# adrelino/mv-lm-icp

Hardware: NVIDIA H100
Metric: ICP iterations/sec (corr+LM) (higher is better)
Workload: dtype f64

## Files before the change

### mv_lm_icp_b200/csrc/lm_step.cuh

```cuda
#pragma once
#include <cuda_runtime.h>
#include "../../include/mvicp.h"
#include "se3_math.cuh"
#include "types.cuh"

namespace mv {

constexpr int STEP_THREADS = 512;
constexpr int EOUT = 160;

struct LmState {
  mvicp_lm_options opt;
  int32_t param, cost_kind, robust, M, E, F, n, G;
  int32_t phase, done, termination, iteration, n_success, n_invalid, n_evals, n_solves, reuse_diagonal, nonrigid;
  double radius, decrease_factor, x_cost, cand_cost, x_norm, initial_cost, model_cost_change, step_norm, gmax;
};

struct NormalLayout {
  const int32_t* col;
  const int32_t* hb_ptr; const int32_t* hb_row; const int32_t* hb_col; const int32_t* hc_edge; const int32_t* hc_sub; int32_t n_hblocks;
  const int32_t* gb_ptr; const int32_t* gc_edge; const int32_t* gc_side;
  const int32_t* rlast; const int32_t* rfirst;
  const int32_t* rowbase;
  double *Lg, *rhs;
  int32_t l_in_smem;
  double* poses16;
  volatile int32_t* host_flag;
  int32_t seq;
};

struct LmWork {
  LmState* S;
  const EdgeDev* edges;
  const double* eout;
  volatile int* peer_flags;
  int32_t world, xseq;
  double* x;
  double* cand;
  Rt* Rt_eval;
  double* K_eval;
  FrameGen* G_eval;
  NormalLayout lay;
  double *H, *g, *Hc, *gc, *scale, *diag, *step;
  long long* prof;
};

struct LmProblem {
  LmState* S;
  const int32_t* frame;
  const int32_t* edge;
  NormalLayout lay;
  double *H, *g, *Hc, *gc, *scale, *diag, *step;
};

__device__ __forceinline__ double block_sum(double v, double* red) {
  __syncthreads();
  const int lane = threadIdx.x & 31, wid = threadIdx.x >> 5;
#pragma unroll
  for (int o = 16; o > 0; o >>= 1) v += __shfl_down_sync(0xffffffffu, v, o);
  if (lane == 0) red[wid] = v;
  __syncthreads();
  if (threadIdx.x == 0) { double s = 0; for (int w = 0; w < STEP_THREADS / 32; ++w) s += red[w]; red[32] = s; }
  __syncthreads();
  return red[32];
}
__device__ __forceinline__ double block_max(double v, double* red) {
  __syncthreads();
  const int lane = threadIdx.x & 31, wid = threadIdx.x >> 5;
#pragma unroll
  for (int o = 16; o > 0; o >>= 1) v = fmax(v, __shfl_down_sync(0xffffffffu, v, o));
  if (lane == 0) red[wid] = v;
  __syncthreads();
  if (threadIdx.x == 0) { double s = 0; for (int w = 0; w < STEP_THREADS / 32; ++w) s = fmax(s, red[w]); red[32] = s; }
  __syncthreads();
  return red[32];
}

__device__ __forceinline__ void gather_blocks(const NormalLayout& l, const double* eout, int n, double* H) {
  for (int idx = threadIdx.x; idx < l.n_hblocks * 36; idx += blockDim.x) {
    const int b = idx / 36, r = idx - 36 * b, i = r / 6, j = r - 6 * i;
    double s = 0;
    for (int c = l.hb_ptr[b]; c < l.hb_ptr[b + 1]; ++c) {
      const int e = l.hc_edge[c], sub = l.hc_sub[c];
      s += eout[(size_t)EOUT * e + (6 * (sub >> 1) + i) * 12 + 6 * (sub & 1) + j];
    }
    H[(size_t)(l.hb_row[b] + i) * n + l.hb_col[b] + j] = s;
  }
}
__device__ __forceinline__ void gather_gradient(const NormalLayout& l, const double* eout, int M, double* g) {
  for (int idx = threadIdx.x; idx < M * 6; idx += blockDim.x) {
    const int f = idx / 6, i = idx - 6 * f;
    if (l.col[f] < 0) continue;
    double s = 0;
    for (int c = l.gb_ptr[f]; c < l.gb_ptr[f + 1]; ++c) s += eout[(size_t)EOUT * l.gc_edge[c] + 144 + 6 * l.gc_side[c] + i];
    g[l.col[f] + i] = s;
  }
}
__device__ __forceinline__ double edge_cost_sum(const double* eout, int E, double* red, const int32_t* edge = nullptr) {
  double s = 0.0;
  for (int e = threadIdx.x; e < E; e += blockDim.x) s += eout[(size_t)EOUT * (edge ? edge[e] : e) + 156];
  return block_sum(s, red);
}
template <typename State> __device__ __forceinline__ void copy_state(State* dst, const State* src) {
  for (int i = threadIdx.x; i < (int)(sizeof(State) / sizeof(int32_t)); i += blockDim.x)
    reinterpret_cast<int32_t*>(dst)[i] = reinterpret_cast<const int32_t*>(src)[i];
  __syncthreads();
}
__device__ __forceinline__ void publish_step(const NormalLayout& l, bool done) {
  __threadfence();
  l.host_flag[l.seq & 7] = (l.seq << 1) | (done ? 1 : 0);
  __threadfence_system();
}

__global__ void lm_init_kernel(LmWork w) {
  LmState* S = w.S;
  const int f = blockIdx.x * blockDim.x + threadIdx.x;
  if (f >= S->M) return;
  double x[7] = {0, 0, 0, 0, 0, 0, 0};
  param_of_pose(S->param, w.lay.poses16 + 16 * f, x);
  if (S->param != PARAM_AA) {
    const double n2 = x[0] * x[0] + x[1] * x[1] + x[2] * x[2] + x[3] * x[3];
    if (!(fabs(n2 - 1.0) <= 1e-9)) atomicExch(&S->nonrigid, 1);
  }
  Rt a; Rt_of_param(S->param, x, &a);
  double K[36]; tangent_map(S->param, x, &a, K);
  for (int i = 0; i < 7; ++i) { w.x[7 * f + i] = x[i]; w.cand[7 * f + i] = x[i]; }
  w.Rt_eval[f] = a;
  for (int i = 0; i < 36; ++i) w.K_eval[36 * f + i] = K[i];
  if (w.G_eval && S->param != PARAM_AA) frame_general(S->param, x, &w.G_eval[f]);
}

__device__ __forceinline__ void chol_factor_diag(double* L, const int32_t* rb, int j0, double* dinv, volatile int* s_ok, int lane) {
  double D[6][6], inv[6];
#pragma unroll
  for (int i = 0; i < 6; ++i)
#pragma unroll
    for (int k = 0; k <= i; ++k) D[i][k] = L[rb[j0 + i] + j0 + k];
  bool okb = true;
#pragma unroll
  for (int k = 0; k < 6; ++k) {
    double d = D[k][k];
#pragma unroll
    for (int m = 0; m < k; ++m) d -= D[k][m] * D[k][m];
    if (!(d > 0.0) || !isfinite(d)) okb = false;
    inv[k] = rsqrt(d); D[k][k] = d * inv[k];
#pragma unroll
    for (int i = k + 1; i < 6; ++i) {
      double v = D[i][k];
#pragma unroll
      for (int m = 0; m < k; ++m) v -= D[i][m] * D[k][m];
      D[i][k] = v * inv[k];
    }
  }
  __syncwarp();
  if (lane == 0) {
    if (!okb) *s_ok = 0;
#pragma unroll
    for (int i = 0; i < 6; ++i) {
#pragma unroll
      for (int k = 0; k <= i; ++k) L[rb[j0 + i] + j0 + k] = D[i][k];
      dinv[j0 + i] = inv[i];
    }
  }
}

__device__ bool chol_solve(double* L, const int32_t* __restrict__ rowbase, int n, double* scratch, double* dinv, double* y,
                           const int32_t* __restrict__ rlast, const int32_t* __restrict__ rfirst, long long* prof = nullptr) {
  const int T = blockDim.x, tid = threadIdx.x, lane = tid & 31, wid = tid >> 5, nw = T >> 5;
  int32_t* s_rfirst = reinterpret_cast<int32_t*>(scratch);
  int32_t* s_rlast = s_rfirst + n;
  int32_t* rb = s_rlast + n;
  volatile int* s_ok = reinterpret_cast<volatile int*>(rb + n + 1);
  for (int i = tid; i < n; i += T) { s_rfirst[i] = rfirst[i]; s_rlast[i] = rlast[i]; }
  for (int i = tid; i <= n; i += T) rb[i] = rowbase[i];
  if (tid == 0) *s_ok = 1;
  __syncthreads();
  const int NB = n / 6;
  if (wid == 0) chol_factor_diag(L, rb, 0, dinv, s_ok, lane);
  __syncthreads();
  long long t_panel = 0, t_ahead = 0, t_bar = 0;
  for (int J = 0; J < NB; ++J) {
    if (!*s_ok) return false;
    const long long c0 = prof ? clock64() : 0;
    const int j0 = 6 * J;
    const int rl = s_rlast[j0 + 5];
    const int nrows = rl - (j0 + 5) + 1;
    for (int q = tid; q < nrows; q += T) {
      const int r = (q == nrows - 1) ? n : j0 + 6 + q;
      if (r < n && s_rfirst[r] > j0 + 5) continue;
      double* row = L + rb[r] + j0;
      double v[6];
#pragma unroll
      for (int k = 0; k < 6; ++k) {
        double a = row[k];
#pragma unroll
        for (int m = 0; m < k; ++m) a -= v[m] * L[rb[j0 + k] + j0 + m];
        v[k] = a * dinv[j0 + k];
      }
#pragma unroll
      for (int k = 0; k < 6; ++k) row[k] = v[k];
    }
    const long long c1 = prof ? clock64() : 0;
    __syncthreads();
    const long long c2 = prof ? clock64() : 0;
    const bool next = J + 1 < NB;
    if (wid == 0 && next) {
      const int b0 = j0 + 6;
      if (lane < 21 && s_rfirst[b0] <= j0 + 5) {
        int i = 0, rem = lane; while (rem > i) { rem -= i + 1; ++i; }
        const int k = rem;
        double* row = L + rb[b0 + i]; const double* lc = L + rb[b0 + k] + j0;
        double a = row[b0 + k];
#pragma unroll
        for (int m = 0; m < 6; ++m) a -= row[j0 + m] * lc[m];
        row[b0 + k] = a;
      }
      __syncwarp();
      chol_factor_diag(L, rb, b0, dinv, s_ok, lane);
    } else {
      const int w0 = next ? 1 : 0, wn = next ? nw - 1 : nw;
      const int qfirst = next ? 6 : 0;
      for (int q = qfirst + (wid - w0); q < nrows; q += wn) {
        const int r = (q == nrows - 1) ? n : j0 + 6 + q;
        if (r < n && s_rfirst[r] > j0 + 5) continue;
        double* row = L + rb[r];
        double lr[6];
#pragma unroll
        for (int k = 0; k < 6; ++k) lr[k] = row[j0 + k];
        const int cend = min(r, rl);
        for (int c = j0 + 6 + lane; c <= cend; c += 32) {
          if (s_rfirst[c] > j0 + 5) continue;
          const double* lc = L + rb[c] + j0;
          double a = row[c];
#pragma unroll
          for (int k = 0; k < 6; ++k) a -= lr[k] * lc[k];
          row[c] = a;
        }
      }
    }
    const long long c3 = prof ? clock64() : 0;
    __syncthreads();
    if (prof) { const long long c4 = clock64(); t_panel += c1 - c0; t_ahead += c3 - c2; t_bar += (c2 - c1) + (c4 - c3); }
  }
  if (prof && tid == 0) { prof[8] = t_panel; prof[9] = t_ahead; prof[10] = t_bar; }
  if (!*s_ok) return false;
  for (int i = tid; i < n; i += T) y[i] = L[rb[n] + i];
  __syncthreads();
  if (wid == 0) {
    for (int J = NB - 1; J >= 0; --J) {
      const int j0 = 6 * J;
      double x[6];
#pragma unroll
      for (int k = 5; k >= 0; --k) {
        double a = y[j0 + k];
#pragma unroll
        for (int m = k + 1; m < 6; ++m) a -= L[rb[j0 + m] + j0 + k] * x[m];
        x[k] = a * dinv[j0 + k];
      }
      __syncwarp();
#pragma unroll
      for (int k = 0; k < 6; ++k) if (lane == k) y[j0 + k] = x[k];
      for (int i = s_rfirst[j0] + lane; i < j0; i += 32) {
        double a = y[i];
#pragma unroll
        for (int k = 0; k < 6; ++k) a -= L[rb[j0 + k] + i] * x[k];
        y[i] = a;
      }
      __syncwarp();
    }
  }
  __syncthreads();
  return true;
}

template <bool COMP>
__device__ __forceinline__ void lm_step_body(const LmWork& w, const LmProblem& p) {
  extern __shared__ double smem[];
  __shared__ double red[40];
  __shared__ int s_flag;
  if (p.S->done) { if (!COMP && threadIdx.x == 0) publish_step(w.lay, true); return; }
  const int tid = threadIdx.x, T = blockDim.x;
  __shared__ LmState s_state;
  copy_state(&s_state, p.S);
  LmState* S = &s_state;
  const int n = S->n, M = S->M, E = S->E, param = S->param;
  const NormalLayout& lay = p.lay;
  auto gf = [&](int f) { return COMP ? p.frame[f] : f; };
  long long* prof = w.prof ? w.prof + 16 * (w.lay.seq & 3) : nullptr;
#define MV_STAMP(i) do { if (prof && tid == 0) prof[i] = clock64(); } while (0)
  MV_STAMP(0);
  if (w.peer_flags) {
    if (tid < w.world) {
      const long long t0 = clock64();
      while (w.peer_flags[tid] - w.xseq < 0) {
        if (clock64() - t0 > 4000000000LL) { S->nonrigid = 2; break; }
      }
    }
    __syncthreads();
  }
  double* colj = smem; double* dg = smem + 2 * (S->n + 1);
  double* L = lay.l_in_smem ? smem + 3 * (S->n + 1) : lay.Lg;

  gather_blocks(lay, w.eout, n, p.Hc);
  gather_gradient(lay, w.eout, M, p.gc);
  __syncthreads();
  const double eval_cost = edge_cost_sum(w.eout, E, red, COMP ? p.edge : nullptr);

  MV_STAMP(1);
  bool take = false;
  if (tid == 0) {
    s_flag = 0;
    S->n_evals += 1;
    if (!isfinite(eval_cost)) {
      if (S->phase == 0) { S->done = 1; S->termination = MVICP_TERM_EVAL_FAILURE; }
      else {
        S->n_invalid += 1;
        if (S->n_invalid >= S->opt.max_num_consecutive_invalid_steps) { S->done = 1; S->termination = MVICP_TERM_INVALID_STEPS; }
        S->radius = S->radius / S->decrease_factor; S->decrease_factor *= 2.0; S->reuse_diagonal = 1;
      }
    } else if (S->phase == 0) {
      S->x_cost = eval_cost; S->initial_cost = eval_cost; s_flag = 1;
    } else {
      S->cand_cost = eval_cost;
      if (S->step_norm <= S->opt.parameter_tolerance * (S->x_norm + S->opt.parameter_tolerance)) {
        S->done = 1; S->termination = MVICP_TERM_PARAMETER_TOLERANCE;
      } else if (fabs(S->x_cost - eval_cost) <= S->opt.function_tolerance * S->x_cost) {
        S->done = 1; S->termination = MVICP_TERM_FUNCTION_TOLERANCE;
      } else {
        const double rho = (S->x_cost - eval_cost) / S->model_cost_change;
        if (rho > S->opt.min_relative_decrease) {
          s_flag = 1; S->n_success += 1; S->x_cost = eval_cost;
          const double q = 2.0 * rho - 1.0;
          S->radius = fmin(S->opt.max_trust_region_radius, S->radius / fmax(1.0 / 3.0, 1.0 - q * q * q));
          S->decrease_factor = 2.0; S->reuse_diagonal = 0;
        } else {
          S->radius = S->radius / S->decrease_factor; S->decrease_factor *= 2.0; S->reuse_diagonal = 1;
          if (S->radius < S->opt.min_trust_region_radius) { S->done = 1; S->termination = MVICP_TERM_MIN_RADIUS; }
        }
      }
    }
  }
  __syncthreads();
  take = s_flag != 0;
  if (take) {
    for (int idx = tid; idx < lay.n_hblocks * 36; idx += T) {
      const int b = idx / 36, r = idx - 36 * b, i = r / 6, j = r - 6 * i;
      const size_t at = (size_t)(lay.hb_row[b] + i) * n + lay.hb_col[b] + j;
      p.H[at] = p.Hc[at];
    }
    for (int idx = tid; idx < n; idx += T) p.g[idx] = p.gc[idx];
    for (int idx = tid; idx < M * 7; idx += T) { const int at = COMP ? 7 * gf(idx / 7) + idx % 7 : idx; w.x[at] = w.cand[at]; }
    __syncthreads();
    if (S->phase == 0)
      for (int j = tid; j < n; j += T) p.scale[j] = S->opt.jacobi_scaling ? 1.0 / (1.0 + sqrt(p.H[(size_t)j * n + j])) : 1.0;
    double xs = 0.0, gm = 0.0;
    for (int f = tid; f < M; f += T) {
      if (lay.col[f] < 0) continue;
      const int G = S->G;
      double xf[7], ng[6], xp[7];
      for (int i = 0; i < G; ++i) { xf[i] = w.x[7 * gf(f) + i]; xs += xf[i] * xf[i]; }
      for (int i = 0; i < 6; ++i) ng[i] = -p.g[lay.col[f] + i];
      param_plus(param, xf, ng, xp);
      for (int i = 0; i < G; ++i) gm = fmax(gm, fabs(xf[i] - xp[i]));
    }
    xs = block_sum(xs, red);
    gm = block_max(gm, red);
    if (tid == 0) {
      S->x_norm = sqrt(xs); S->gmax = gm;
      if (gm <= S->opt.gradient_tolerance) { S->done = 1; S->termination = MVICP_TERM_GRADIENT_TOLERANCE; }
      if (S->phase == 0) { S->phase = 1; S->iteration = 0; S->reuse_diagonal = 0; }
    }
    __syncthreads();
  }

  MV_STAMP(2);
  while (!S->done) {
    __syncthreads();
    if (S->iteration >= S->opt.max_num_iterations) {
      __syncthreads();
      if (tid == 0) { S->done = 1; S->termination = MVICP_TERM_MAX_ITERATIONS; }
      __syncthreads();
      break;
    }
    const int reuse = S->reuse_diagonal;
    const double radius = S->radius;
    __syncthreads();
    if (!reuse)
      for (int j = tid; j < n; j += T) {
        const double d = p.scale[j] * p.scale[j] * p.H[(size_t)j * n + j];
        p.diag[j] = fmin(fmax(d, S->opt.min_lm_diagonal), S->opt.max_lm_diagonal);
      }
    __syncthreads();
    for (int i = tid >> 5; i < n; i += T >> 5) {
      const double si = p.scale[i];
      const int rbi = lay.rowbase[i];
      for (int j = lay.rfirst[i] + (tid & 31); j <= i; j += 32) {
        double v = si * p.H[(size_t)i * n + j] * p.scale[j];
        if (i == j) { const double ldg = sqrt(p.diag[i] / radius); v += ldg * ldg; }
        L[rbi + j] = v;
      }
    }
    { const int rbn = lay.rowbase[n]; for (int j = tid; j < n; j += T) L[rbn + j] = p.scale[j] * p.g[j]; }
    __syncthreads();
    MV_STAMP(3);
    bool ok = chol_solve(L, lay.rowbase, n, colj, dg, lay.rhs, lay.rlast, lay.rfirst, prof);
    MV_STAMP(4);
    double bad = 0.0;
    if (ok) for (int j = tid; j < n; j += T) if (!isfinite(lay.rhs[j])) bad = 1.0;
    bad = block_sum(bad, red);
    ok = ok && (bad == 0.0);
    double mcc = 0.0;
    if (ok) {
      for (int j = tid; j < n; j += T) p.step[j] = -lay.rhs[j];
      __syncthreads();
      double acc = 0.0;
      for (int i = tid; i < n; i += T) {
        const double y = lay.rhs[i];
        acc += 0.5 * (y * p.scale[i] * p.g[i] + (p.diag[i] / radius) * y * y);
      }
      mcc = block_sum(acc, red);
    }
    const bool valid = ok && (mcc > 0.0);
    __syncthreads();
    if (tid == 0) {
      S->iteration += 1; S->n_solves += 1; S->reuse_diagonal = 1; S->model_cost_change = mcc;
      if (!valid) {
        S->n_invalid += 1;
        if (S->n_invalid >= S->opt.max_num_consecutive_invalid_steps) { S->done = 1; S->termination = MVICP_TERM_INVALID_STEPS; }
        S->radius = S->radius / S->decrease_factor; S->decrease_factor *= 2.0;
      } else S->n_invalid = 0;
    }
    __syncthreads();
    if (!valid) continue;
    double sn = 0.0;
    for (int f = tid; f < M; f += T) {
      const int G = S->G, g_f = gf(f);
      double xf[7], d[6], xp[7] = {0, 0, 0, 0, 0, 0, 0};
      for (int i = 0; i < 7; ++i) xf[i] = w.x[7 * g_f + i];
      if (lay.col[f] >= 0) {
        for (int i = 0; i < 6; ++i) d[i] = p.step[lay.col[f] + i] * p.scale[lay.col[f] + i];
        param_plus(param, xf, d, xp);
        for (int i = 0; i < G; ++i) sn += (xf[i] - xp[i]) * (xf[i] - xp[i]);
      } else for (int i = 0; i < 7; ++i) xp[i] = xf[i];
      for (int i = 0; i < 7; ++i) w.cand[7 * g_f + i] = xp[i];
      Rt a; Rt_of_param(param, xp, &a);
      w.Rt_eval[g_f] = a;
      double K[36]; tangent_map(param, xp, &a, K);
      for (int i = 0; i < 36; ++i) w.K_eval[36 * g_f + i] = K[i];
      if (w.G_eval && param != PARAM_AA) frame_general(param, xp, &w.G_eval[g_f]);
    }
    sn = block_sum(sn, red);
    MV_STAMP(5);
    if (tid == 0) S->step_norm = sqrt(sn);
    __syncthreads();
    break;
  }
  __syncthreads();
  if (S->done) {
    for (int f = tid; f < M; f += T) {
      double xf[7]; for (int i = 0; i < 7; ++i) xf[i] = w.x[7 * gf(f) + i];
      pose_of_param(param, xf, w.lay.poses16 + 16 * gf(f));
    }
  }
  __syncthreads();
  copy_state(p.S, &s_state);
  MV_STAMP(6);
  if (!COMP && tid == 0) publish_step(w.lay, S->done);
  MV_STAMP(7);
#undef MV_STAMP
}

__global__ void __launch_bounds__(STEP_THREADS) lm_step_kernel(LmWork w) {
  const LmProblem p{w.S, nullptr, nullptr, w.lay, w.H, w.g, w.Hc, w.gc, w.scale, w.diag, w.step};
  lm_step_body<false>(w, p);
}

__global__ void __launch_bounds__(STEP_THREADS) lm_step_components_kernel(LmWork w, const LmProblem* __restrict__ probs, unsigned int* ticket) {
  __shared__ LmProblem s_prob;
  copy_state(&s_prob, probs + blockIdx.x);
  lm_step_body<true>(w, s_prob);
  __shared__ int s_last;
  __syncthreads();
  if (threadIdx.x == 0) { __threadfence(); s_last = atomicAdd(ticket, 1u) == gridDim.x - 1; }
  __syncthreads();
  if (!s_last) return;
  __threadfence();
  int open = 0;
  for (int k = threadIdx.x; k < (int)gridDim.x; k += blockDim.x) open |= *(volatile const int*)&probs[k].S->done == 0;
  open = __syncthreads_count(open);
  if (threadIdx.x == 0) { *ticket = 0u; publish_step(w.lay, open == 0); }
}

}
```

### mv_lm_icp_b200/csrc/mvicp.cu

```cuda
#include <cuda_runtime.h>
#include <nccl.h>
#ifdef __linux__
#include <sched.h>
#endif
#include <algorithm>
#include <atomic>
#include <cmath>
#include <cstdarg>
#include <cstdio>
#include <cstdlib>
#include <cstring>
#include <limits>
#include <numeric>
#include <string>
#include <thread>
#include <vector>

#include "../../include/mvicp.h"
#include "closed.cuh"
#include "compact.cuh"
#include "device_io.cuh"
#include "far.cuh"
#include "g2o.cuh"
#include "knn.cuh"
// ... 3 lines not shown
#include "se3_math.cuh"
#include "select.cuh"
#include "types.cuh"

using namespace mv;

static thread_local std::string g_err;
static int fail(int code, const char* fmt, ...) {
  char buf[512];
  va_list ap; va_start(ap, fmt); vsnprintf(buf, sizeof buf, fmt, ap); va_end(ap);
  g_err = buf;
  return code;
}
#define CU(call)                                                                                              \
  do {                                                                                                        \
    cudaError_t e_ = (call);                                                                                  \
    if (e_ != cudaSuccess) return fail(MVICP_ERR_CUDA, "%s:%d %s: %s", __FILE__, __LINE__, #call, cudaGetErrorString(e_)); \
  } while (0)
#define NC(call)                                                                                              \
  do {                                                                                                        \
    ncclResult_t r_ = (call);                                                                                 \
    if (r_ != ncclSuccess) return fail(MVICP_ERR_NCCL, "%s:%d %s: %s", __FILE__, __LINE__, #call, ncclGetErrorString(r_)); \
  } while (0)
#define RET(call) do { int r__ = (call); if (r__ != MVICP_OK) return r__; } while (0)

struct DevBuf {
  void* p = nullptr; size_t cap = 0;
  DevBuf() = default;
  DevBuf(const DevBuf&) = delete;
  DevBuf& operator=(const DevBuf&) = delete;
  ~DevBuf() { release(); }
  int reserve(size_t bytes) {
    if (bytes <= cap) return MVICP_OK;
    if (p) cudaFree(p);
    p = nullptr; cap = 0;
    CU(cudaMalloc(&p, bytes ? bytes : 16));
    cap = bytes ? bytes : 16;
    return MVICP_OK;
  }
  void release() { if (p) cudaFree(p); p = nullptr; cap = 0; }
  template <typename T> T* as() const { return reinterpret_cast<T*>(p); }
};

struct mvicp_ctx {
  int device = 0, flags = 0;
  cudaStream_t stream = nullptr; bool own_stream = false;
  int rank = 0, world = 1; ncclComm_t comm = nullptr;
  void* xbuf = nullptr; void* peer_x[MAX_PEERS] = {}; bool p2p_ok = false; int32_t xseq = 0;
  static constexpr int X_ECAP = 4096;
  int M = 0; bool f32 = true; bool nor_f32 = true; bool have_normals = true;
  std::vector<void*> nor_dbl;
  float normals_ms = 0.f;
  std::vector<int64_t> n_pts;
  std::vector<FrameDev> h_frames;
  std::vector<void*> frame_allocs;
  DevBuf d_obb;
  int seeded_rounds = 0;
  DevBuf d_single;
  DevBuf d_prof;
  DevBuf d_tile_count, d_tile_off, d_edge_off, d_recs;
  bool obb_ready = false;
  int last_lm_iters = 1 << 20;
  DevBuf d_frames, d_poses;
  std::vector<uint8_t> fixed;
  std::vector<double> h_poses;
  int E = 0;
  std::vector<EdgeDev> h_edges;
  std::vector<int32_t> edge_owner;
  DevBuf d_edges, d_xf, d_corr, d_d2, d_count, d_sel, d_hist, d_weight, d_median, d_selcand, d_selcand_n;
  DevBuf d_sel_cnt;
  DevBuf d_sel_win;
  DevBuf d_certs, d_cert_cnt;
  DevBuf d_todo, d_todo_n;
  bool cert_valid = false;
  int64_t cert_rounds = 0;
  bool sel_valid = false;
  int64_t sel_guess_rounds = 0;
  DevBuf d_knn_tiles, d_eval_tiles, d_edge_tile_begin, d_partial;
  int n_knn_tiles = 0, n_eval_tiles = 0, eval_tile_len = EVAL_TILE;
  int64_t total_slots = 0;
  bool have_corr = false;
  bool nonrigid = false;
  std::vector<float> h_weight; std::vector<unsigned long long> h_count;
  DevBuf d_state, d_x, d_cand, d_Rt, d_K, d_col, d_H, d_g, d_Hc, d_gc, d_scale, d_diag, d_L, d_rhs, d_step,
      d_eout, d_hb_ptr, d_hb_row, d_hb_col, d_hc_edge, d_hc_sub, d_gb_ptr, d_gc_edge, d_gc_side, d_posegather, d_rlast, d_rfirst, d_rowbase, d_gen;
  int64_t l_size = 0;
  int n_free = 0;
  NormalLayout lay{};
  std::vector<int32_t> h_col;
  void* h_state = nullptr;
  volatile int32_t* h_flag = nullptr; volatile int32_t* d_flag = nullptr;
  std::vector<uint8_t> lm_key; uint32_t graph_gen = 0;
  DevBuf d_cmp_i32, d_cmp_f64, d_cmp_prob, d_cmp_state, d_cmp_ticket;
  std::vector<uint8_t> cmp_key;
  std::vector<int32_t> cmp_of_frame;
  std::vector<int32_t> cmp_prob;
  std::vector<int32_t> cmp_M, cmp_E, cmp_n;
  int n_cmp = 0, n_prob = 0; size_t cmp_dyn = 0, cmp_edge_map = 0;
  DevBuf d_g2o_state, d_g2o_x, d_g2o_ev, d_g2o_nop, d_g2o_chi, d_g2o_trace, d_g2o_tiles, d_g2o_tile_begin, d_g2o_cnt;
  int64_t g2o_trials = 0;
  mvicp_stats stats{};
  cudaEvent_t ev[8]{};
  std::vector<cudaEvent_t> eval_ev;
  int eval_ev_used = 0;
  bool ev_knn = false, ev_lm = false;
  float lm_eval_acc = 0.f;
  DevBuf d_cpq, d_cpr;
  DevBuf d_set_win, d_set_bad;
  DevBuf d_knn_nor;
};

static inline int owner_of(const mvicp_ctx* c, int frame) { return (int)(((int64_t)frame * c->world) / std::max(1, c->M)); }
static void assign_edge_owners(mvicp_ctx* c) {
  const int E = c->E;
  c->edge_owner.assign(E, -1);
  int64_t total = 0;
  for (int e = 0; e < E; ++e) if (!c->fixed[c->h_edges[e].src]) total += c->n_pts[c->h_edges[e].src];
  int64_t before = 0;
  for (int e = 0; e < E; ++e) {
    const int s = c->h_edges[e].src;
    if (c->fixed[s]) continue;
    const int64_t n = c->n_pts[s];
    c->edge_owner[e] = total > 0 ? (int)std::min<int64_t>(c->world - 1, ((2 * before + n) * c->world) / (2 * total)) : 0;
    before += n;
  }
}

#include "tree_build.h"
#include "tree_gpu.cuh"

extern "C" { static int refresh_after_fixed_change(mvicp_ctx* c); }

static bool poses_nonrigid(const double* poses16, int M) {
  for (int f = 0; f < M; ++f) {
    Rt a; pose16_to_Rt(poses16 + 16 * f, &a);
    double q[4]; quat_of_matrix(a.R, q);
    const double n2 = q[0] * q[0] + q[1] * q[1] + q[2] * q[2] + q[3] * q[3];
    if (!(std::fabs(n2 - 1.0) <= 1e-9)) return true;
  }
  return false;
}

static unsigned host_workers() {
  unsigned n = std::max(1u, std::thread::hardware_concurrency());
#ifdef __linux__
  cpu_set_t set; CPU_ZERO(&set);
  if (sched_getaffinity(0, sizeof set, &set) == 0) { const int k = CPU_COUNT(&set); if (k > 0) n = std::min<unsigned>(n, (unsigned)k); }
  if (FILE* f = std::fopen("/sys/fs/cgroup/cpu.max", "r")) {
    char q[32]; long long period = 0;
    if (std::fscanf(f, "%31s %lld", q, &period) == 2 && std::strcmp(q, "max") != 0 && period > 0) {
      const long long quota = std::atoll(q);
      if (quota > 0) n = std::min<unsigned>(n, (unsigned)std::max<long long>(1, quota / period));
    }
    std::fclose(f);
  }
#endif
  return std::max(1u, n);
}

static int finish_set_frames(mvicp_ctx* c, int M) {
  if (c->f32 && c->nor_f32)
    for (int f = 0; f < M; ++f) {
      FrameDev& fr = c->h_frames[f];
      if (!fr.nor_o) continue;
      void* d_pn = nullptr;
      CU(cudaMalloc(&d_pn, sizeof(float4) * 2 * (size_t)fr.n)); c->frame_allocs.push_back(d_pn);
      pack_pn_kernel<<<(fr.n + 255) / 256, 256, 0, c->stream>>>((const float4*)fr.pts_o, (const float4*)fr.nor_o, fr.n, (float4*)d_pn);
// ... 956 lines not shown
        v = c->h_flag[want & 7];
        if ((v >> 1) != want) { CU(cudaGetLastError()); return fail(MVICP_ERR_CUDA, "%s step %d never reported", what, want); }
        break;
      }
    }
    ++seen;
    if ((v & 1) != 0 || seen > max_evals) break;
  }
  return MVICP_OK;
}

static int read_back_solve(mvicp_ctx* c, void* state, const void* d_state, size_t bytes) {
  CU(cudaEventRecord(c->ev[4], c->stream));
  CU(cudaMemcpyAsync(state, d_state, bytes, cudaMemcpyDeviceToHost, c->stream));
  CU(cudaMemcpyAsync(c->h_poses.data(), c->d_poses.p, sizeof(double) * 16 * c->M, cudaMemcpyDeviceToHost, c->stream));
  CU(cudaStreamSynchronize(c->stream));
  CU(cudaGetLastError());
  c->ev_lm = true;
  return MVICP_OK;
}

static int refresh_if_fixed_changed(mvicp_ctx* c) {
  bool stale = false;
  for (int e = 0; e < c->E; ++e) if ((c->edge_owner[e] < 0) != (c->fixed[c->h_edges[e].src] != 0)) stale = true;
  if (!stale) return MVICP_OK;
  if (c->world > 1) return fail(MVICP_ERR_STATE, "sharded run: frame 0 was free when the edges were distributed; fix it (mvicp_set_poses) before mvicp_correspond");
  return refresh_after_fixed_change(c);
}

template <typename Solve>
static int run_pairwise(const mvicp_config* cfg, const double* src, const double* dst, const double* nor, int64_t n, double* pose16_out,
                        Solve&& solve) {
  mvicp_ctx* c = nullptr;
  RET(mvicp_create(cfg, &c));
  const double* pts[2] = {dst, src}; const double* nrs[2] = {nor, nor};
  const int64_t np[2] = {n, n};
  int rc = mvicp_set_frames(c, 2, pts, nor ? nrs : nullptr, np);
  const int32_t es = 1, ed = 0;
  if (rc == MVICP_OK) rc = mvicp_set_graph(c, 1, &es, &ed);
  if (rc == MVICP_OK) {
    std::vector<int32_t> id(n); std::iota(id.begin(), id.end(), 0);
    rc = mvicp_set_edge(c, 0, id.data(), id.data(), n, 1.0f);
  }
  if (rc == MVICP_OK) rc = solve(c);
  std::vector<double> poses(32);
  if (rc == MVICP_OK) rc = mvicp_get_poses(c, poses.data());
  if (rc == MVICP_OK) std::memcpy(pose16_out, poses.data() + 16, sizeof(double) * 16);
  const std::string keep = g_err;
  mvicp_destroy(c);
  g_err = keep;
  return rc;
}

static void summary_of_state(const LmState& st, mvicp_lm_summary* s) {
  s->termination = st.termination; s->num_iterations = st.iteration; s->num_successful_steps = st.n_success;
  s->num_evaluations = st.n_evals; s->num_linear_solves = st.n_solves; s->reserved = 0;
  s->initial_cost = st.initial_cost; s->final_cost = st.x_cost;
}
static void summary_no_unknowns(mvicp_lm_summary* s) { std::memset(s, 0, sizeof *s); s->termination = MVICP_TERM_GRADIENT_TOLERANCE; }

extern "C" {
int mvicp_optimize(mvicp_ctx* c, int32_t param, int32_t cost, int32_t robust, const mvicp_lm_options* opt_in, mvicp_lm_summary* summary) {
  if (!c || !c->M || !c->E) return fail(MVICP_ERR_STATE, "mvicp_optimize: frames and graph must be set first");
  if (param < 0 || param > 2 || cost < 0 || cost > 2) return fail(MVICP_ERR_INVALID, "mvicp_optimize: bad param/cost");
  if (cost != COST_P2P && !c->have_normals) return fail(MVICP_ERR_INVALID, "point-to-plane needs normals for every frame");
  RET(check_lm_options(opt_in, "mvicp_optimize"));
  CU(cudaSetDevice(c->device));
  const int M = c->M, E = c->E;
  c->fixed[0] = 1;
  c->h_col.assign(M, -1); int n = 0;
  for (int f = 0; f < M; ++f) if (!c->fixed[f]) { c->h_col[f] = n; n += 6; }
  c->n_free = n / 6;
  mvicp_lm_options opt; if (opt_in) opt = *opt_in; else mvicp_default_lm_options(&opt);
  if (n == 0) {
    if (summary) summary_no_unknowns(summary);
    return MVICP_OK;
  }
  RET(refresh_if_fixed_changed(c));
  std::vector<uint8_t> key(c->fixed); key.push_back((uint8_t)(c->graph_gen & 0xff)); key.push_back((uint8_t)((c->graph_gen >> 8) & 0xff));
  if (key != c->lm_key) {
    RET(c->d_state.reserve(sizeof(LmState)));
    RET(c->d_x.reserve(sizeof(double) * 7 * M)); RET(c->d_cand.reserve(sizeof(double) * 7 * M));
    RET(c->d_Rt.reserve(sizeof(Rt) * M)); RET(c->d_K.reserve(sizeof(double) * 36 * M));
    RET(c->d_Hc.reserve(sizeof(double) * n * n)); RET(c->d_gc.reserve(sizeof(double) * n)); RET(c->d_scale.reserve(sizeof(double) * n));
    RET(c->d_diag.reserve(sizeof(double) * n)); RET(c->d_step.reserve(sizeof(double) * n));
    CU(cudaMemsetAsync(c->d_Hc.p, 0, sizeof(double) * (size_t)n * n, c->stream));
    std::vector<uint8_t> active(E);
    for (int e = 0; e < E; ++e) active[e] = !c->fixed[c->h_edges[e].src];
    RET(build_normal_layout(c, n, active));
    c->lm_key = key;
  }
  LmState st; std::memset(&st, 0, sizeof st);
  st.opt = opt; st.param = param; st.cost_kind = cost; st.robust = robust ? 1 : 0; st.M = M; st.E = E; st.F = n / 6; st.n = n;
  st.G = ambient_size(param); st.radius = opt.initial_trust_region_radius; st.decrease_factor = 2.0;
  std::memcpy(c->h_state, &st, sizeof st);
  CU(cudaMemcpyAsync(c->d_state.p, c->h_state, sizeof st, cudaMemcpyHostToDevice, c->stream));

  LmWork w{};
  w.S = c->d_state.as<LmState>(); w.edges = c->d_edges.as<EdgeDev>(); w.eout = c->d_eout.as<double>();
  if (std::getenv("MVICP_STEP_PROFILE")) { RET(c->d_prof.reserve(sizeof(long long) * 64)); w.prof = c->d_prof.as<long long>(); }
  c->nonrigid = poses_nonrigid(c->h_poses.data(), M);
  const bool general = c->nonrigid && param != PARAM_AA;
  if (general) { RET(c->d_gen.reserve(sizeof(FrameGen) * M)); RET(c->d_partial.reserve(sizeof(double) * GBLK * std::max<size_t>(1, c->n_eval_tiles))); }
  w.G_eval = general ? c->d_gen.as<FrameGen>() : nullptr;
  w.x = c->d_x.as<double>(); w.cand = c->d_cand.as<double>(); w.Rt_eval = c->d_Rt.as<Rt>(); w.K_eval = c->d_K.as<double>();
  w.lay = c->lay; w.lay.poses16 = c->d_poses.as<double>();
  w.H = c->d_H.as<double>(); w.g = c->d_g.as<double>(); w.Hc = c->d_Hc.as<double>(); w.gc = c->d_gc.as<double>();
  w.scale = c->d_scale.as<double>(); w.diag = c->d_diag.as<double>(); w.step = c->d_step.as<double>();

  CU(cudaEventRecord(c->ev[3], c->stream));
  lm_init_kernel<<<(M + 63) / 64, 64, 0, c->stream>>>(w);
  c->stats.kernel_launches += 1;
  const int64_t max_evals = (int64_t)opt.max_num_iterations + 2;
  const bool use_p2p = c->comm && c->world > 1 && c->p2p_ok && E <= mvicp_ctx::X_ECAP;
  const DoneGate done_flag{&w.S->done, nullptr, 0};
  auto eval = [&]() {
    if (general) { if (c->f32) launch_eval_general<true>(c, param, cost, st.robust, done_flag); else launch_eval_general<false>(c, param, cost, st.robust, done_flag); }
    else if (c->f32) launch_eval<true>(c, cost, st.robust, done_flag); else launch_eval<false>(c, cost, st.robust, done_flag);
  };
  auto step = [&](size_t dyn) -> int {
    PeerTable pt; std::memset(&pt, 0, sizeof pt); pt.world = 1; pt.rank = 0;
    double* eout_local = c->d_eout.as<double>();
    unsigned int* xcounter = nullptr;
    int xs = 0;
    if (use_p2p) {
      xs = ++c->xseq;
      const size_t half = (size_t)mvicp_ctx::X_ECAP * EOUT;
      pt.world = c->world; pt.rank = c->rank;
      for (int p = 0; p < c->world; ++p) {
        pt.eout[p] = (double*)c->peer_x[p] + (size_t)(xs & 1) * half;
        pt.flags[p] = (volatile int*)((double*)c->peer_x[p] + 2 * half);
      }
      eout_local = pt.eout[c->rank];
      xcounter = (unsigned int*)((double*)c->xbuf + 2 * half) + 32;
    }
    if (general)
      lm_edge_general_kernel<<<E, EDGE_THREADS, 0, c->stream>>>(c->d_edges.as<EdgeDev>(), c->d_edge_tile_begin.as<int32_t>(),
                                                                c->d_partial.as<double>(), eout_local, done_flag, pt, xs, xcounter);
    else
      lm_edge_kernel<<<E, EDGE_THREADS, 0, c->stream>>>(c->d_edges.as<EdgeDev>(), c->d_edge_tile_begin.as<int32_t>(), c->d_partial.as<double>(),
                                                        cost == COST_P2PLANE ? NBLK_PLANE : NBLK, c->d_Rt.as<Rt>(), c->d_K.as<double>(),
                                                        eout_local, done_flag, pt, xs, xcounter);
    if (c->comm && c->world > 1 && !use_p2p)
      NC(ncclAllReduce(c->d_eout.p, c->d_eout.p, (size_t)EOUT * E, ncclDouble, ncclSum, c->comm, c->stream));
    w.eout = eout_local; w.peer_flags = use_p2p ? pt.flags[c->rank] : nullptr; w.world = c->world; w.xseq = xs;
    lm_step_kernel<<<1, STEP_THREADS, dyn, c->stream>>>(w);
    c->stats.kernel_launches += (c->n_eval_tiles ? 1 : 0) + 2;
    return MVICP_OK;
  };
  RET(run_steps(c, lm_step_kernel, n, max_evals, "LM", w.lay, eval, step));
  if (c->comm && c->world > 1 && !use_p2p) {
    const int chunk = (M + c->world - 1) / c->world;
    RET(c->d_posegather.reserve(sizeof(double) * 16 * (size_t)chunk * c->world * 2));
    double* sendb = c->d_posegather.as<double>();
    double* recvb = sendb + (size_t)16 * chunk * c->world;
    CU(cudaMemsetAsync(sendb, 0, sizeof(double) * 16 * chunk, c->stream));
    int f0 = -1, f1 = -1;
    for (int f = 0; f < M; ++f) if (owner_of(c, f) == c->rank) { if (f0 < 0) f0 = f; f1 = f; }
    if (f0 >= 0) CU(cudaMemcpyAsync(sendb, c->d_poses.as<double>() + 16 * f0, sizeof(double) * 16 * (f1 - f0 + 1), cudaMemcpyDeviceToDevice, c->stream));
    NC(ncclAllGather(sendb, recvb, (size_t)16 * chunk, ncclDouble, c->comm, c->stream));
    for (int r = 0; r < c->world; ++r) {
      int a = -1, b = -1;
      for (int f = 0; f < M; ++f) if (owner_of(c, f) == r) { if (a < 0) a = f; b = f; }
      if (a >= 0) CU(cudaMemcpyAsync(c->d_poses.as<double>() + 16 * a, recvb + (size_t)16 * chunk * r, sizeof(double) * 16 * (b - a + 1), cudaMemcpyDeviceToDevice, c->stream));
    }
  }
  RET(read_back_solve(c, c->h_state, c->d_state.p, sizeof st));
  std::memcpy(&st, c->h_state, sizeof st);
  c->last_lm_iters = st.iteration;
  if (summary) summary_of_state(st, summary);
  if (st.nonrigid == 2) return fail(MVICP_ERR_NCCL, "a peer rank never delivered its pair matrices (peer-memory exchange timed out)");
  if (st.nonrigid && !general)
    return fail(MVICP_ERR_NONRIGID, "a pose's quaternion is not unit (non-rigid Isometry) but the unit-quaternion LM path was run");
  if (!st.done) return fail(MVICP_ERR_STATE, "LM loop did not terminate within %lld evaluations", (long long)max_evals);
  return MVICP_OK;
}

}
static int graph_components(const mvicp_ctx* c, std::vector<int32_t>& comp) {
  std::vector<int32_t> up(c->M);
  std::iota(up.begin(), up.end(), 0);
  auto root = [&](int f) { while (up[f] != f) f = up[f] = up[up[f]]; return f; };
  for (const EdgeDev& e : c->h_edges) {
    const int a = root(e.src), b = root(e.dst);
    if (a != b) up[std::max(a, b)] = std::min(a, b);
  }
  comp.assign(c->M, -1);
  int n = 0;
  for (int f = 0; f < c->M; ++f) { const int r = root(f); comp[f] = r == f ? n++ : comp[r]; }
  return n;
}

static int build_component_layouts(mvicp_ctx* c, const std::vector<uint8_t>& key) {
  const int M = c->M, E = c->E;
  const int K = c->n_cmp = graph_components(c, c->cmp_of_frame);
  std::vector<std::vector<int32_t>> fr(K), ed(K);
  for (int f = 0; f < M; ++f) fr[c->cmp_of_frame[f]].push_back(f);
  for (int e = 0; e < E; ++e) ed[c->cmp_of_frame[c->h_edges[e].src]].push_back(e);
  std::vector<uint8_t> active(E);
  for (int e = 0; e < E; ++e) active[e] = !c->fixed[c->h_edges[e].src];
  c->h_col.assign(M, -1);
  c->cmp_prob.assign(K, -1); c->cmp_M.clear(); c->cmp_E.clear(); c->cmp_n.clear();
  std::vector<LayoutPlan> plans; std::vector<int32_t> pc;
  for (int k = 0; k < K; ++k) {
    int n = 0;
    for (int f : fr[k]) if (!c->fixed[f]) { c->h_col[f] = n; n += 6; }
    if (!n) continue;
    c->cmp_prob[k] = (int32_t)plans.size();
    plans.emplace_back();
    RET(plan_normal_layout(c, fr[k], ed[k], n, active, plans.back()));
    pc.push_back(k); c->cmp_n.push_back(n);
    c->cmp_M.push_back((int32_t)fr[k].size()); c->cmp_E.push_back((int32_t)ed[k].size());
  }
  const int P = c->n_prob = (int)plans.size();
  if (!P) { c->cmp_key = key; return MVICP_OK; }
  std::vector<int32_t> blob;
  auto put = [&](const std::vector<int32_t>& v) { const size_t o = blob.size(); blob.insert(blob.end(), v.begin(), v.end()); return o; };
  struct Off { size_t frame, edge, col, hb_ptr, hb_row, hb_col, hc_edge, hc_sub, gb_ptr, gc_edge, gc_side, rlast, rfirst, rowbase; };
  std::vector<Off> io(P);
  for (int q = 0; q < P; ++q) {
    const LayoutPlan& pl = plans[q];
    io[q] = Off{put(fr[pc[q]]), put(ed[pc[q]]), put(pl.col), put(pl.hb_ptr), put(pl.hb_row), put(pl.hb_col), put(pl.hc_edge), put(pl.hc_sub),
                put(pl.gb_ptr), put(pl.gc_edge), put(pl.gc_side), put(pl.rlast), put(pl.rfirst), put(pl.rowbase)};
  }
  std::vector<int32_t> prob_of_edge(E);
  for (int e = 0; e < E; ++e) prob_of_edge[e] = c->cmp_prob[c->cmp_of_frame[c->h_edges[e].src]];
  c->cmp_edge_map = put(prob_of_edge);
  std::vector<size_t> fo(P + 1, 0);
  for (int q = 0; q < P; ++q) { const size_t n = c->cmp_n[q]; fo[q + 1] = fo[q] + 2 * n * n + 6 * n + (size_t)plans[q].l_size; }
  RET(c->d_cmp_i32.reserve(sizeof(int32_t) * blob.size()));
  RET(c->d_cmp_f64.reserve(sizeof(double) * fo[P]));
  RET(c->d_cmp_prob.reserve(sizeof(LmProblem) * P));
  RET(c->d_cmp_state.reserve(sizeof(LmState) * (P + 1)));
  RET(c->d_cmp_ticket.reserve(sizeof(unsigned int)));
  const int32_t* ib = c->d_cmp_i32.as<int32_t>();
  std::vector<LmProblem> probs(P);
  size_t dyn = 0;
  for (int q = 0; q < P; ++q) {
    const int n = c->cmp_n[q]; const Off& o = io[q];
    LmProblem& p = probs[q];
    std::memset(&p, 0, sizeof p);
    p.S = c->d_cmp_state.as<LmState>() + q;
    p.frame = ib + o.frame; p.edge = ib + o.edge;
    NormalLayout& l = p.lay;
    l.col = ib + o.col;
    l.hb_ptr = ib + o.hb_ptr; l.hb_row = ib + o.hb_row; l.hb_col = ib + o.hb_col; l.hc_edge = ib + o.hc_edge; l.hc_sub = ib + o.hc_sub;
    l.n_hblocks = (int32_t)plans[q].hb_row.size();
    l.gb_ptr = ib + o.gb_ptr; l.gc_edge = ib + o.gc_edge; l.gc_side = ib + o.gc_side;
    l.rlast = ib + o.rlast; l.rfirst = ib + o.rfirst; l.rowbase = ib + o.rowbase;
    double* d = c->d_cmp_f64.as<double>() + fo[q];
    p.H = d; d += (size_t)n * n; p.Hc = d; d += (size_t)n * n;
    p.g = d; d += n; p.gc = d; d += n; p.scale = d; d += n; p.diag = d; d += n; p.step = d; d += n; l.rhs = d; d += n;
    l.Lg = d;
    const size_t vec = sizeof(double) * 3 * (size_t)(n + 1), lb = sizeof(double) * (size_t)plans[q].l_size;
    l.l_in_smem = lb + vec <= 220 * 1024 ? 1 : 0;
    dyn = std::max(dyn, vec + (l.l_in_smem ? lb : 0));
  }
  c->cmp_dyn = dyn;
  CU(cudaMemcpyAsync(c->d_cmp_i32.p, blob.data(), sizeof(int32_t) * blob.size(), cudaMemcpyHostToDevice, c->stream));
  CU(cudaMemcpyAsync(c->d_cmp_prob.p, probs.data(), sizeof(LmProblem) * P, cudaMemcpyHostToDevice, c->stream));
  CU(cudaMemsetAsync(c->d_cmp_f64.p, 0, sizeof(double) * fo[P], c->stream));
  CU(cudaMemsetAsync(c->d_cmp_ticket.p, 0, sizeof(unsigned int), c->stream));
  CU(cudaStreamSynchronize(c->stream));
  c->cmp_key = key;
  return MVICP_OK;
}

extern "C" {
int mvicp_get_components(mvicp_ctx* c, int32_t* n_components, int32_t* component_of_frame) {
  if (!c || !n_components) return fail(MVICP_ERR_INVALID, "mvicp_get_components: bad arguments");
  if (!c->M) return fail(MVICP_ERR_STATE, "mvicp_get_components: frames must be set first");
  std::vector<int32_t> comp;
  *n_components = graph_components(c, comp);
  if (component_of_frame) std::memcpy(component_of_frame, comp.data(), sizeof(int32_t) * c->M);
  return MVICP_OK;
}

int mvicp_optimize_components(mvicp_ctx* c, int32_t param, int32_t cost, int32_t robust, const mvicp_lm_options* opt_in,
                              mvicp_lm_summary* summaries) {
  if (!c || !c->M || !c->E) return fail(MVICP_ERR_STATE, "mvicp_optimize_components: frames and graph must be set first");
  if (param < 0 || param > 2 || cost < 0 || cost > 2) return fail(MVICP_ERR_INVALID, "mvicp_optimize_components: bad param/cost");
  if (cost != COST_P2P && !c->have_normals) return fail(MVICP_ERR_INVALID, "point-to-plane needs normals for every frame");
  if (c->world > 1) return fail(MVICP_ERR_STATE, "mvicp_optimize_components: the component solve runs on one GPU; this context is sharded");
  RET(check_lm_options(opt_in, "mvicp_optimize_components"));
  CU(cudaSetDevice(c->device));
  const int M = c->M, E = c->E;
  {
    std::vector<int32_t> comp;
    std::vector<uint8_t> seen(graph_components(c, comp), 0);
    for (int f = 0; f < M; ++f) if (!seen[comp[f]]) { seen[comp[f]] = 1; c->fixed[f] = 1; }
  }
  mvicp_lm_options opt; if (opt_in) opt = *opt_in; else mvicp_default_lm_options(&opt);
  if (std::all_of(c->fixed.begin(), c->fixed.end(), [](uint8_t v) { return v != 0; })) {
    if (summaries) { int32_t K = 0; RET(mvicp_get_components(c, &K, nullptr)); for (int k = 0; k < K; ++k) summary_no_unknowns(summaries + k); }
    return MVICP_OK;
  }
  RET(refresh_if_fixed_changed(c));
  std::vector<uint8_t> key(c->fixed); key.push_back((uint8_t)(c->graph_gen & 0xff)); key.push_back((uint8_t)((c->graph_gen >> 8) & 0xff));
  if (key != c->cmp_key) RET(build_component_layouts(c, key));
  const int P = c->n_prob;
  std::vector<LmState> st(P + 1);
  std::memset(st.data(), 0, sizeof(LmState) * (P + 1));
  for (int q = 0; q <= P; ++q) {
    LmState& s = st[q];
    s.opt = opt; s.param = param; s.cost_kind = cost; s.robust = robust ? 1 : 0; s.G = ambient_size(param);
    if (q == P) { s.M = M; s.E = E; continue; }
    s.M = c->cmp_M[q]; s.E = c->cmp_E[q]; s.n = c->cmp_n[q]; s.F = s.n / 6;
    s.radius = opt.initial_trust_region_radius; s.decrease_factor = 2.0;
  }
  LmState* dS = c->d_cmp_state.as<LmState>();
  CU(cudaMemcpyAsync(dS, st.data(), sizeof(LmState) * (P + 1), cudaMemcpyHostToDevice, c->stream));
  RET(c->d_x.reserve(sizeof(double) * 7 * M)); RET(c->d_cand.reserve(sizeof(double) * 7 * M));
  RET(c->d_Rt.reserve(sizeof(Rt) * M)); RET(c->d_K.reserve(sizeof(double) * 36 * M));
  RET(c->d_eout.reserve(sizeof(double) * EOUT * E));
  c->nonrigid = poses_nonrigid(c->h_poses.data(), M);
  const bool general = c->nonrigid && param != PARAM_AA;
  if (general) { RET(c->d_gen.reserve(sizeof(FrameGen) * M)); RET(c->d_partial.reserve(sizeof(double) * GBLK * std::max<size_t>(1, c->n_eval_tiles))); }
  LmWork w{};
  w.S = dS + P; w.edges = c->d_edges.as<EdgeDev>(); w.eout = c->d_eout.as<double>(); w.world = 1;
  w.x = c->d_x.as<double>(); w.cand = c->d_cand.as<double>(); w.Rt_eval = c->d_Rt.as<Rt>(); w.K_eval = c->d_K.as<double>();
  w.G_eval = general ? c->d_gen.as<FrameGen>() : nullptr;
  w.lay.poses16 = c->d_poses.as<double>(); w.lay.host_flag = c->d_flag;
  const LmProblem* probs = c->d_cmp_prob.as<LmProblem>();
  unsigned int* ticket = c->d_cmp_ticket.as<unsigned int>();

  CU(cudaEventRecord(c->ev[3], c->stream));
  lm_init_kernel<<<(M + 63) / 64, 64, 0, c->stream>>>(w);
  c->stats.kernel_launches += 1;
  const int64_t max_evals = (int64_t)opt.max_num_iterations + 2;
  const DoneGate gate{&dS[0].done, c->d_cmp_i32.as<int32_t>() + c->cmp_edge_map, (int32_t)(sizeof(LmState) / sizeof(int))};
  auto eval = [&]() {
    if (general) { if (c->f32) launch_eval_general<true>(c, param, cost, st[0].robust, gate); else launch_eval_general<false>(c, param, cost, st[0].robust, gate); }
    else if (c->f32) launch_eval<true>(c, cost, st[0].robust, gate); else launch_eval<false>(c, cost, st[0].robust, gate);
  };
  auto step = [&](size_t) -> int {
// ... 463 lines not shown
```

Baseline: 563.9.

## Overlap Cholesky panel with diagonal factor via named barriers; drop Hc/gc staging

The blocked Cholesky now has warp 0 solve the next block's six panel rows, update the diagonal block with shuffles and factor it from registers, while the other warps do the remaining panel rows. A named barrier (bar.arrive/bar.sync 1) replaces one full __syncthreads per block column. Separately, the candidate Hessian and gradient are gathered straight into H and g only when a step is accepted, which removes the Hc/gc buffers and the copy between them. This cuts barriers and memory traffic in exchange for more complex synchronization, and the gather runs on each accepted step rather than on every evaluation.

Measured after the change: 563.9, median of 6. Within noise of the previous version (-0.0%).

```diff
diff --git a/mv_lm_icp_b200/csrc/lm_step.cuh b/mv_lm_icp_b200/csrc/lm_step.cuh
--- a/mv_lm_icp_b200/csrc/lm_step.cuh
+++ b/mv_lm_icp_b200/csrc/lm_step.cuh
@@ -41,7 +41,7 @@
   double* K_eval;
   FrameGen* G_eval;
   NormalLayout lay;
-  double *H, *g, *Hc, *gc, *scale, *diag, *step;
+  double *H, *g, *scale, *diag, *step;
   long long* prof;
 };
 
@@ -50,7 +50,7 @@
   const int32_t* frame;
   const int32_t* edge;
   NormalLayout lay;
-  double *H, *g, *Hc, *gc, *scale, *diag, *step;
+  double *H, *g, *scale, *diag, *step;
 };
 
 __device__ __forceinline__ double block_sum(double v, double* red) {
@@ -130,12 +130,12 @@
   if (w.G_eval && S->param != PARAM_AA) frame_general(S->param, x, &w.G_eval[f]);
 }
 
-__device__ __forceinline__ void chol_factor_diag(double* L, const int32_t* rb, int j0, double* dinv, volatile int* s_ok, int lane) {
-  double D[6][6], inv[6];
+__device__ __forceinline__ void chol_factor_diag(double a, double (&D)[6][6], double (&inv)[6], double* L, const int32_t* rb, int j0,
+                                                 double* dinv, volatile int* s_ok, int lane) {
 #pragma unroll
   for (int i = 0; i < 6; ++i)
 #pragma unroll
-    for (int k = 0; k <= i; ++k) D[i][k] = L[rb[j0 + i] + j0 + k];
+    for (int k = 0; k <= i; ++k) D[i][k] = __shfl_sync(0xffffffffu, a, i * (i + 1) / 2 + k);
   bool okb = true;
 #pragma unroll
   for (int k = 0; k < 6; ++k) {
@@ -162,6 +162,34 @@
       dinv[j0 + i] = inv[i];
     }
   }
+}
+
+__device__ __forceinline__ void cta_arrive1() {
+#ifdef __CUDA_ARCH__
+  asm volatile("bar.arrive 1, %0;" ::"r"(blockDim.x) : "memory");
+#else
+  __syncthreads();
+#endif
+}
+__device__ __forceinline__ void cta_wait1() {
+#ifdef __CUDA_ARCH__
+  asm volatile("bar.sync 1, %0;" ::"r"(blockDim.x) : "memory");
+#else
+  __syncthreads();
+#endif
+}
+__device__ __forceinline__ void chol_panel_row(double* L, const int32_t* rb, int r, int j0, const double* dinv) {
+  double* row = L + rb[r] + j0;
+  double v[6];
+#pragma unroll
+  for (int k = 0; k < 6; ++k) {
+    double a = row[k];
+#pragma unroll
+    for (int m = 0; m < k; ++m) a -= v[m] * L[rb[j0 + k] + j0 + m];
+    v[k] = a * dinv[j0 + k];
+  }
+#pragma unroll
+  for (int k = 0; k < 6; ++k) row[k] = v[k];
 }
 
 __device__ bool chol_solve(double* L, const int32_t* __restrict__ rowbase, int n, double* scratch, double* dinv, double* y,
@@ -176,7 +204,10 @@
   if (tid == 0) *s_ok = 1;
   __syncthreads();
   const int NB = n / 6;
-  if (wid == 0) chol_factor_diag(L, rb, 0, dinv, s_ok, lane);
+  int ti = 0, tk = lane;
+  while (tk > ti) { tk -= ti + 1; ++ti; }
+  double D[6][6], inv[6];
+  if (wid == 0) chol_factor_diag(lane < 21 ? L[rb[ti] + tk] : 0.0, D, inv, L, rb, 0, dinv, s_ok, lane);
   __syncthreads();
   long long t_panel = 0, t_ahead = 0, t_bar = 0;
   for (int J = 0; J < NB; ++J) {
@@ -185,42 +216,57 @@
     const int j0 = 6 * J;
     const int rl = s_rlast[j0 + 5];
     const int nrows = rl - (j0 + 5) + 1;
-    for (int q = tid; q < nrows; q += T) {
-      const int r = (q == nrows - 1) ? n : j0 + 6 + q;
-      if (r < n && s_rfirst[r] > j0 + 5) continue;
-      double* row = L + rb[r] + j0;
-      double v[6];
-#pragma unroll
-      for (int k = 0; k < 6; ++k) {
-        double a = row[k];
-#pragma unroll
-        for (int m = 0; m < k; ++m) a -= v[m] * L[rb[j0 + k] + j0 + m];
-        v[k] = a * dinv[j0 + k];
-      }
-#pragma unroll
-      for (int k = 0; k < 6; ++k) row[k] = v[k];
-    }
-    const long long c1 = prof ? clock64() : 0;
-    __syncthreads();
-    const long long c2 = prof ? clock64() : 0;
     const bool next = J + 1 < NB;
-    if (wid == 0 && next) {
+    if (!next) {
+      for (int q = tid; q < nrows; q += T) {
+        const int r = (q == nrows - 1) ? n : j0 + 6 + q;
+        if (r < n && s_rfirst[r] > j0 + 5) continue;
+        chol_panel_row(L, rb, r, j0, dinv);
+      }
+      const long long c1 = prof ? clock64() : 0;
+      __syncthreads();
+      if (prof) { t_panel += c1 - c0; t_bar += clock64() - c1; }
+      break;
+    }
+    long long c1 = 0, c3 = 0;
+    if (wid == 0) {
       const int b0 = j0 + 6;
-      if (lane < 21 && s_rfirst[b0] <= j0 + 5) {
-        int i = 0, rem = lane; while (rem > i) { rem -= i + 1; ++i; }
-        const int k = rem;
-        double* row = L + rb[b0 + i]; const double* lc = L + rb[b0 + k] + j0;
-        double a = row[b0 + k];
-#pragma unroll
-        for (int m = 0; m < 6; ++m) a -= row[j0 + m] * lc[m];
-        row[b0 + k] = a;
+      const bool link = s_rfirst[b0] <= j0 + 5;
+      double v[6] = {0, 0, 0, 0, 0, 0};
+      if (link && lane < 6) {
+        double* row = L + rb[b0 + lane] + j0;
+#pragma unroll
+        for (int k = 0; k < 6; ++k) {
+          double a = row[k];
+#pragma unroll
+          for (int m = 0; m < k; ++m) a -= v[m] * D[k][m];
+          v[k] = a * inv[k];
+        }
+#pragma unroll
+        for (int k = 0; k < 6; ++k) row[k] = v[k];
       }
       __syncwarp();
-      chol_factor_diag(L, rb, b0, dinv, s_ok, lane);
+      cta_arrive1();
+      if (prof) c1 = clock64();
+      double a = lane < 21 ? L[rb[b0 + ti] + b0 + tk] : 0.0;
+      if (link) {
+#pragma unroll
+        for (int m = 0; m < 6; ++m) {
+          const double li = __shfl_sync(0xffffffffu, v[m], ti), lk = __shfl_sync(0xffffffffu, v[m], tk);
+          a -= li * lk;
+        }
+      }
+      chol_factor_diag(a, D, inv, L, rb, b0, dinv, s_ok, lane);
+      if (prof) c3 = clock64();
     } else {
-      const int w0 = next ? 1 : 0, wn = next ? nw - 1 : nw;
-      const int qfirst = next ? 6 : 0;
-      for (int q = qfirst + (wid - w0); q < nrows; q += wn) {
+      const int qs = min(6, nrows - 1);
+      for (int q = qs + tid - 32; q < nrows; q += T - 32) {
+        const int r = (q == nrows - 1) ? n : j0 + 6 + q;
+        if (r < n && s_rfirst[r] > j0 + 5) continue;
+        chol_panel_row(L, rb, r, j0, dinv);
+      }
+      cta_wait1();
+      for (int q = 6 + (wid - 1); q < nrows; q += nw - 1) {
         const int r = (q == nrows - 1) ? n : j0 + 6 + q;
         if (r < n && s_rfirst[r] > j0 + 5) continue;
         double* row = L + rb[r];
@@ -238,9 +284,8 @@
         }
       }
     }
-    const long long c3 = prof ? clock64() : 0;
-    __syncthreads();
-    if (prof) { const long long c4 = clock64(); t_panel += c1 - c0; t_ahead += c3 - c2; t_bar += (c2 - c1) + (c4 - c3); }
+    __syncthreads();
+    if (prof) { const long long c4 = clock64(); t_panel += c1 - c0; t_ahead += c3 - c1; t_bar += c4 - c3; }
   }
   if (prof && tid == 0) { prof[8] = t_panel; prof[9] = t_ahead; prof[10] = t_bar; }
   if (!*s_ok) return false;
@@ -301,9 +346,6 @@
   double* colj = smem; double* dg = smem + 2 * (S->n + 1);
   double* L = lay.l_in_smem ? smem + 3 * (S->n + 1) : lay.Lg;
 
-  gather_blocks(lay, w.eout, n, p.Hc);
-  gather_gradient(lay, w.eout, M, p.gc);
-  __syncthreads();
   const double eval_cost = edge_cost_sum(w.eout, E, red, COMP ? p.edge : nullptr);
 
   MV_STAMP(1);
@@ -343,12 +385,8 @@
   __syncthreads();
   take = s_flag != 0;
   if (take) {
-    for (int idx = tid; idx < lay.n_hblocks * 36; idx += T) {
-      const int b = idx / 36, r = idx - 36 * b, i = r / 6, j = r - 6 * i;
-      const size_t at = (size_t)(lay.hb_row[b] + i) * n + lay.hb_col[b] + j;
-      p.H[at] = p.Hc[at];
-    }
-    for (int idx = tid; idx < n; idx += T) p.g[idx] = p.gc[idx];
+    gather_blocks(lay, w.eout, n, p.H);
+    gather_gradient(lay, w.eout, M, p.g);
     for (int idx = tid; idx < M * 7; idx += T) { const int at = COMP ? 7 * gf(idx / 7) + idx % 7 : idx; w.x[at] = w.cand[at]; }
     __syncthreads();
     if (S->phase == 0)
@@ -471,7 +509,7 @@
 }
 
 __global__ void __launch_bounds__(STEP_THREADS) lm_step_kernel(LmWork w) {
-  const LmProblem p{w.S, nullptr, nullptr, w.lay, w.H, w.g, w.Hc, w.gc, w.scale, w.diag, w.step};
+  const LmProblem p{w.S, nullptr, nullptr, w.lay, w.H, w.g, w.scale, w.diag, w.step};
   lm_step_body<false>(w, p);
 }
 
diff --git a/mv_lm_icp_b200/csrc/mvicp.cu b/mv_lm_icp_b200/csrc/mvicp.cu
--- a/mv_lm_icp_b200/csrc/mvicp.cu
+++ b/mv_lm_icp_b200/csrc/mvicp.cu
@@ -109,7 +109,7 @@
   bool have_corr = false;
   bool nonrigid = false;
   std::vector<float> h_weight; std::vector<unsigned long long> h_count;
-  DevBuf d_state, d_x, d_cand, d_Rt, d_K, d_col, d_H, d_g, d_Hc, d_gc, d_scale, d_diag, d_L, d_rhs, d_step,
+  DevBuf d_state, d_x, d_cand, d_Rt, d_K, d_col, d_H, d_g, d_scale, d_diag, d_L, d_rhs, d_step,
       d_eout, d_hb_ptr, d_hb_row, d_hb_col, d_hc_edge, d_hc_sub, d_gb_ptr, d_gc_edge, d_gc_side, d_posegather, d_rlast, d_rfirst, d_rowbase, d_gen;
   int64_t l_size = 0;
   int n_free = 0;
@@ -1232,9 +1232,8 @@
     RET(c->d_state.reserve(sizeof(LmState)));
     RET(c->d_x.reserve(sizeof(double) * 7 * M)); RET(c->d_cand.reserve(sizeof(double) * 7 * M));
     RET(c->d_Rt.reserve(sizeof(Rt) * M)); RET(c->d_K.reserve(sizeof(double) * 36 * M));
-    RET(c->d_Hc.reserve(sizeof(double) * n * n)); RET(c->d_gc.reserve(sizeof(double) * n)); RET(c->d_scale.reserve(sizeof(double) * n));
+    RET(c->d_scale.reserve(sizeof(double) * n));
     RET(c->d_diag.reserve(sizeof(double) * n)); RET(c->d_step.reserve(sizeof(double) * n));
-    CU(cudaMemsetAsync(c->d_Hc.p, 0, sizeof(double) * (size_t)n * n, c->stream));
     std::vector<uint8_t> active(E);
     for (int e = 0; e < E; ++e) active[e] = !c->fixed[c->h_edges[e].src];
     RET(build_normal_layout(c, n, active));
@@ -1255,7 +1254,7 @@
   w.G_eval = general ? c->d_gen.as<FrameGen>() : nullptr;
   w.x = c->d_x.as<double>(); w.cand = c->d_cand.as<double>(); w.Rt_eval = c->d_Rt.as<Rt>(); w.K_eval = c->d_K.as<double>();
   w.lay = c->lay; w.lay.poses16 = c->d_poses.as<double>();
-  w.H = c->d_H.as<double>(); w.g = c->d_g.as<double>(); w.Hc = c->d_Hc.as<double>(); w.gc = c->d_gc.as<double>();
+  w.H = c->d_H.as<double>(); w.g = c->d_g.as<double>();
   w.scale = c->d_scale.as<double>(); w.diag = c->d_diag.as<double>(); w.step = c->d_step.as<double>();
 
   CU(cudaEventRecord(c->ev[3], c->stream));
@@ -1377,7 +1376,7 @@
   for (int e = 0; e < E; ++e) prob_of_edge[e] = c->cmp_prob[c->cmp_of_frame[c->h_edges[e].src]];
   c->cmp_edge_map = put(prob_of_edge);
   std::vector<size_t> fo(P + 1, 0);
-  for (int q = 0; q < P; ++q) { const size_t n = c->cmp_n[q]; fo[q + 1] = fo[q] + 2 * n * n + 6 * n + (size_t)plans[q].l_size; }
+  for (int q = 0; q < P; ++q) { const size_t n = c->cmp_n[q]; fo[q + 1] = fo[q] + n * n + 5 * n + (size_t)plans[q].l_size; }
   RET(c->d_cmp_i32.reserve(sizeof(int32_t) * blob.size()));
   RET(c->d_cmp_f64.reserve(sizeof(double) * fo[P]));
   RET(c->d_cmp_prob.reserve(sizeof(LmProblem) * P));
@@ -1399,8 +1398,8 @@
     l.gb_ptr = ib + o.gb_ptr; l.gc_edge = ib + o.gc_edge; l.gc_side = ib + o.gc_side;
     l.rlast = ib + o.rlast; l.rfirst = ib + o.rfirst; l.rowbase = ib + o.rowbase;
     double* d = c->d_cmp_f64.as<double>() + fo[q];
-    p.H = d; d += (size_t)n * n; p.Hc = d; d += (size_t)n * n;
-    p.g = d; d += n; p.gc = d; d += n; p.scale = d; d += n; p.diag = d; d += n; p.step = d; d += n; l.rhs = d; d += n;
+    p.H = d; d += (size_t)n * n;
+    p.g = d; d += n; p.scale = d; d += n; p.diag = d; d += n; p.step = d; d += n; l.rhs = d; d += n;
     l.Lg = d;
     const size_t vec = sizeof(double) * 3 * (size_t)(n + 1), lb = sizeof(double) * (size_t)plans[q].l_size;
     l.l_in_smem = lb + vec <= 220 * 1024 ? 1 : 0;
```
